# ApsaraDB/galaxysql

Hardware: AMD Instinct MI355X
Metric: probe_rows_per_s (higher is better)
Workload: dtype int64; 1 GPU; C3_tpch_sf100_q3_join_chain_groupby; customer_rows_per_gpu=15000000, orders_rows_per_gpu=150000000, lineitem_rows_scanned_per_gpu=600000000, lineitem_rows_joined_per_gpu=323601457, groups_last_step=12883243, aggregates=SUM(revenue) f64 + SUM(rev_scaled4) i64 + COUNT(*), exchange=none, parallelism=hash_shuffle_dp1, probe_launches=81

## Files before the change

### galaxysql_amd/csrc/gxhip_agg.inc

```

namespace {

struct __align__(16) AggSlot {
    unsigned long long claim;
    uint32_t gid;
    uint32_t pad;
};

__device__ __host__ static inline uint32_t agg_tag(int32_t h) {
    return ((uint32_t)h << 1) | 1u;
}

struct __align__(16) PackedKey {
    unsigned long long lo, hi;
};

__global__ void k_agg_pack(KeyViews keys, int64_t n, int64_t base,
                           PackedKey *packed, uint8_t *nullmask,
                           int32_t *hashes) {
    for (int64_t r = blockIdx.x * (int64_t)blockDim.x + threadIdx.x; r < n;
         r += (int64_t)gridDim.x * blockDim.x) {
        PackedKey p;
        p.lo = 0; p.hi = 0;
        uint8_t mask = 0;
// ... 103 lines not shown
    DevColView input[GX_MAX_COLS];
    unsigned long long *records;
};

struct AggVal {
    unsigned long long bits;
    int32_t type;
    bool isnull;
};

__device__ static inline int64_t aggval_i64(const AggVal &v) {
    return (int64_t)v.bits;
}
__device__ static inline double aggval_f64(const AggVal &v) {
    return v.type == GX_F64 ? __builtin_bit_cast(double, v.bits)
                            : (double)(int64_t)v.bits;
}

__device__ static inline AggVal agg_load(int32_t func, const DevColView &c,
                                         int64_t r) {
    AggVal v;
    v.bits = 0;
    v.type = c.type;
    v.isnull = false;
    if (func == GX_AGG_COUNT_ROW) return v;
    v.isnull = col_is_null(c, r);
    if (v.isnull || func == GX_AGG_COUNT_COL || c.type == GX_SLICE) return v;
    v.bits = c.type == GX_I32
        ? (unsigned long long)(int64_t)((const int32_t *)c.values)[r]
        : ((const unsigned long long *)c.values)[r];
    return v;
}

__device__ static inline void agg_rmw(int32_t func, unsigned long long *rec,
                                      int32_t val_off, int32_t seen_off,
                                      const AggVal &v) {
    unsigned long long *vp = rec + val_off;
    if (func == GX_AGG_COUNT_ROW) {
        atomicAdd(vp, 1ull);
        return;
    }
    if (v.isnull) return;
    switch (func) {
    case GX_AGG_COUNT_COL:
        atomicAdd(vp, 1ull);
        break;
    case GX_AGG_SUM_I64:
        atomicAdd(vp, v.bits);
        break;
    case GX_AGG_SUM_I64N:
        atomicAdd(vp, v.bits);
        if (seen_off >= 0) rec[seen_off] = 1ull;
        break;
    case GX_AGG_SUM_F64:
        atomicAdd((double *)vp, aggval_f64(v));
        rec[seen_off] = 1ull;
        break;
    case GX_AGG_MIN_I64:
        atomic_min_i64((long long *)vp, (long long)aggval_i64(v));
        rec[seen_off] = 1ull;
        break;
    case GX_AGG_MAX_I64:
        atomic_max_i64((long long *)vp, (long long)aggval_i64(v));
        rec[seen_off] = 1ull;
        break;
    case GX_AGG_MIN_F64:
        atomic_jmin_f64(vp, __builtin_bit_cast(double, v.bits));
        rec[seen_off] = 1ull;
        break;
    case GX_AGG_MAX_F64:
        atomic_jmax_f64(vp, __builtin_bit_cast(double, v.bits));
        rec[seen_off] = 1ull;
        break;
    case GX_AGG_BIT_AND: atomicAnd(vp, v.bits); break;
    case GX_AGG_BIT_OR: atomicOr(vp, v.bits); break;
    case GX_AGG_BIT_XOR: atomicXor(vp, v.bits); break;
    case GX_AGG_AVG_F64:
        atomicAdd((double *)vp, aggval_f64(v));
        atomicAdd(rec + seen_off, 1ull);
        break;
    }
}

__device__ static inline void agg_apply(const AggAccumParams &P, uint32_t gid,
                                        int64_t r) {
    unsigned long long *rec = P.records + (size_t)gid * P.stride;
    for (int a = 0; a < P.n_aggs; a++)
        agg_rmw(P.func[a], rec, P.val_off[a], P.seen_off[a],
                agg_load(P.func[a], P.input[a], r));
}

struct AggInsertParams {
    AggSlot *slots;
    uint32_t mask;
    int use_packed;
    const PackedKey *packed;
    const uint8_t *nullmask;
    KeyViews keystore;
    const int32_t *hashes;
    int64_t base_krow;
    int64_t n;
    uint32_t *overflow;
    int inline_gid;
    uint32_t *ngroups;
    uint32_t *krow_of_gid;
    uint32_t *slot_of_gid;
    uint32_t *slot_of_row;
    int fuse_accum;
    int only_failed;
    AggAccumParams A;
};

#define GX_SLOT_FAIL 0xFFFFFFFFu

__device__ static inline bool agg_rows_equal(const AggInsertParams &P,
                                             int64_t a, int64_t b) {
    if (P.use_packed) return packed_equal(P.packed, P.nullmask, a, b);
    return rows_key_equal(P.keystore, a, P.keystore, b);
}

#define GX_GID_PENDING 0xFFFFFFFFu

__global__ void k_agg_insert(AggInsertParams P) {
    for (int64_t r = blockIdx.x * (int64_t)blockDim.x + threadIdx.x; r < P.n;
         r += (int64_t)gridDim.x * blockDim.x) {
        if (P.only_failed && P.slot_of_row[r] != GX_SLOT_FAIL)
            continue;
        const int64_t krow = P.base_krow + r;
        const uint32_t tag = agg_tag(P.hashes[r]);
        const unsigned long long claim =
            ((unsigned long long)tag << 32) | (uint32_t)(krow + 1);
        uint32_t slot = (uint32_t)gx_mix(P.hashes[r]) & P.mask;
        uint32_t probes = 0;
        bool failed = false;
        while (true) {
            unsigned long long old = P.slots[slot].claim;
            if (old == 0ull)
                old = atomicCAS(&P.slots[slot].claim, 0ull, claim);
            if (old == 0ull) {
                if (P.inline_gid) {
                    uint32_t gid = atomicAdd(P.ngroups, 1u);
                    P.slots[slot].gid = gid;
                    P.krow_of_gid[gid] = (uint32_t)krow;
                    if (P.slot_of_gid)
                        P.slot_of_gid[gid] = slot;
                } else {
                    P.slots[slot].gid = GX_GID_PENDING;
                }
                break;
            }
            if ((uint32_t)(old >> 32) == tag) {
                int64_t owner = (int64_t)(uint32_t)old - 1;
                if (agg_rows_equal(P, owner, krow))
                    break;
            }
            if (++probes > (P.mask < 1023u ? P.mask : 1023u)) {
                *P.overflow = 1u;
                failed = true;
                break;
            }
            slot = (slot + 1) & P.mask;
        }
        if (P.fuse_accum) {
            P.slot_of_row[r] = failed ? GX_SLOT_FAIL : slot;
            if (!failed) agg_apply(P.A, slot, r);
        } else {
// ... 990 lines not shown
```

### galaxysql_amd/csrc/gxhip_groupjoin.inc

```

namespace {

struct __align__(16) GJWideEntry {
    int64_t key;
    uint32_t pos;
    uint32_t used;
    unsigned long long s[2];
};

__global__ void k_gjw_expand(const JoinEntry *entries, int64_t n,
                             DevColView keycol, GJWideEntry *wide,
                             unsigned long long s0, unsigned long long s1) {
    for (int64_t i = blockIdx.x * (int64_t)blockDim.x + threadIdx.x; i < n;
         i += (int64_t)gridDim.x * blockDim.x) {
        JoinEntry e = entries[i];
        GJWideEntry w;
        w.key = ((const int64_t *)keycol.values)[e.pos];
        w.pos = e.pos;
        w.used = 0;
        w.s[0] = s0;
        w.s[1] = s1;
        wide[i] = w;
    }
}
// ... 59 lines not shown
__global__ void k_gjw_unpack(const GJWideEntry *wide, int64_t n,
                             unsigned long long *records, int32_t stride,
                             int32_t off0, int32_t off1, int32_t n_aggs,
                             uint32_t *used) {
    for (int64_t i = blockIdx.x * (int64_t)blockDim.x + threadIdx.x; i < n;
         i += (int64_t)gridDim.x * blockDim.x) {
        GJWideEntry w = wide[i];
        unsigned long long *rec = records + (size_t)w.pos * stride;
        rec[off0] = w.s[0];
        if (n_aggs > 1) rec[off1] = w.s[1];
        if (w.used) atomicOr(&used[w.pos >> 5], 1u << (w.pos & 31));
    }
}

struct GJProbeParams {
    const uint32_t *starts;
    const JoinEntry *entries;
    uint32_t mask;
    int64_t n;
    const int32_t *hashes;
    int fast_i64;
    KeyViews build_keys, probe_keys;
    uint32_t *used;
    unsigned long long *matches;
    AggAccumParams A;
};

__global__ void k_gj_probe(GJProbeParams P) {
    uint32_t n_match = 0;
    for (int64_t i = blockIdx.x * (int64_t)blockDim.x + threadIdx.x; i < P.n;
         i += (int64_t)gridDim.x * blockDim.x) {
        uint32_t b = (uint32_t)gx_mix(P.hashes[i]) & P.mask;
        uint32_t it = P.starts[b], end = P.starts[b + 1];
        int64_t want_key = 0;
        if (P.fast_i64)
            want_key = ((const int64_t *)P.probe_keys.col[0].values)[i];
        for (; it < end; it++) {
            JoinEntry e = P.entries[it];
            bool is_match;
            if (P.fast_i64)
                is_match = (e.key == want_key);
            else
                is_match = ((int32_t)e.key == P.hashes[i]) &&
                           rows_key_equal(P.build_keys, e.pos,
                                          P.probe_keys, i);
            if (!is_match) continue;
            n_match++;
            uint32_t w = 1u << (e.pos & 31);
            if ((P.used[e.pos >> 5] & w) == 0)
                atomicOr(&P.used[e.pos >> 5], w);
            agg_apply(P.A, e.pos, i);
        }
    }
    gj_count_matches(P.matches, n_match);
}

struct GJInlineProbeParams {
    const JoinEntry *table;
    const JoinEntry *entries;
    uint32_t mask;
    int64_t n;
    DevColView probe_key;
    uint32_t *used;
    unsigned long long *matches;
    AggAccumParams A;
};

__global__ void k_gj_probe_inline(GJInlineProbeParams P) {
    uint32_t n_match = 0;
    for (int64_t i = blockIdx.x * (int64_t)blockDim.x + threadIdx.x; i < P.n;
         i += (int64_t)gridDim.x * blockDim.x) {
        if (col_is_null(P.probe_key, i)) continue;
        const int64_t want = ((const int64_t *)P.probe_key.values)[i];
        const uint64_t ebase =
            (uint64_t)((uint32_t)gx_mix(gx_hash_i64(want)) & P.mask) * 4;
        const uint32_t end = P.table[ebase].pad;
        const uint32_t ovf0 = end > 4 ? P.table[ebase + 1].pad : 0u;
        for (uint32_t it = 0; it < end; it++) {
            const JoinEntry e = it < 4 ? P.table[ebase + it]
                                       : P.entries[ovf0 + (it - 4)];
            if (e.key != want) continue;
            n_match++;
            uint32_t w = 1u << (e.pos & 31);
            if ((P.used[e.pos >> 5] & w) == 0)
                atomicOr(&P.used[e.pos >> 5], w);
            agg_apply(P.A, e.pos, i);
        }
    }
    gj_count_matches(P.matches, n_match);
}

__global__ void k_gj_compact(const uint32_t *used, int64_t n, uint32_t *out,
                             uint32_t *counter) {
    __shared__ uint32_t s_rows[4][GX_EMIT_STAGE];
    const int wid = threadIdx.x >> 6;
    const int lane = threadIdx.x & 63;
    uint32_t *stage = s_rows[wid];
    uint32_t cnt = 0;

    auto flush = [&]() {
        if (cnt == 0) return;
        uint32_t base = 0;
        if (lane == 0) base = atomicAdd(counter, cnt);
        base = (uint32_t)__shfl((int)base, 0, 64);
        for (uint32_t k = (uint32_t)lane; k < cnt; k += 64)
            out[base + k] = stage[k];
        cnt = 0;
    };

    const int64_t stride = (int64_t)gridDim.x * blockDim.x;
    for (int64_t i = blockIdx.x * (int64_t)blockDim.x + threadIdx.x;;
         i += stride) {
        bool active = i < n;
        if (!__ballot(active)) break;
        bool want = active && (used[i >> 5] >> (i & 31)) & 1u;
        unsigned long long m = __ballot(want);
        uint32_t add = (uint32_t)__popcll(m);
        if (cnt + add > GX_EMIT_STAGE) flush();
        if (want)
            stage[cnt + (uint32_t)__popcll(m & ((1ull << lane) - 1ull))] =
                (uint32_t)i;
        cnt += add;
    }
    flush();
}

__global__ void k_gj_emit(const unsigned long long *records, int32_t stride,
                          int32_t val_off, int32_t seen_off, int32_t func,
                          const uint32_t *idx, const uint32_t *used,
                          int count_row_null_row, int64_t n,
                          void *out_vals, uint8_t *out_nulls) {
    for (int64_t i = blockIdx.x * (int64_t)blockDim.x + threadIdx.x; i < n;
         i += (int64_t)gridDim.x * blockDim.x) {
        uint32_t g = idx ? idx[i] : (uint32_t)i;
        const unsigned long long *rec = records + (size_t)g * stride;
        bool matched = (used[g >> 5] >> (g & 31)) & 1u;
        bool isnull = seen_off >= 0 && rec[seen_off] == 0ull;
        out_nulls[i] = isnull;
        bool f64 = func == GX_AGG_SUM_F64 || func == GX_AGG_MIN_F64 ||
                   func == GX_AGG_MAX_F64 || func == GX_AGG_AVG_F64;
        unsigned long long v = isnull ? 0ull : rec[val_off];
        if (func == GX_AGG_AVG_F64) {
            ((double *)out_vals)[i] = isnull ? 0.0
                : __builtin_bit_cast(double, v) / (double)rec[seen_off];
        } else if (f64) {
            ((double *)out_vals)[i] = isnull ? 0.0
                : __builtin_bit_cast(double, v);
        } else {
            int64_t x = (int64_t)v;
            if (func == GX_AGG_COUNT_ROW && !matched && count_row_null_row)
                x += 1;
            ((int64_t *)out_vals)[i] = x;
        }
    }
}

struct GJEmitParams {
    const unsigned long long *records;
    int32_t stride;
    const uint32_t *idx;
    const uint32_t *used;
    int count_row_null_row;
    int64_t n;
    int32_t n_keys, n_aggs;
    DevColView key_src[GX_MAX_COLS];
    int32_t key_words[GX_MAX_COLS];
    void *key_vals[GX_MAX_COLS];
    uint8_t *key_nulls[GX_MAX_COLS];
    int32_t func[GX_MAX_COLS];
    int32_t val_off[GX_MAX_COLS];
    int32_t seen_off[GX_MAX_COLS];
    void *agg_vals[GX_MAX_COLS];
    uint8_t *agg_nulls[GX_MAX_COLS];
};

__global__ void k_gj_emit_all(GJEmitParams P) {
    for (int64_t i = blockIdx.x * (int64_t)blockDim.x + threadIdx.x; i < P.n;
         i += (int64_t)gridDim.x * blockDim.x) {
        const uint32_t g = P.idx ? P.idx[i] : (uint32_t)i;
        for (int k = 0; k < P.n_keys; k++) {
            const DevColView &src = P.key_src[k];
            const bool nn = col_is_null(src, g);
            if (P.key_nulls[k]) P.key_nulls[k][i] = nn;
            const int32_t w = P.key_words[k];
            const uint32_t *sv = (const uint32_t *)src.values + (size_t)g * w;
            uint32_t *dv = (uint32_t *)P.key_vals[k] + (size_t)i * w;
            for (int32_t j = 0; j < w; j++) dv[j] = nn ? 0u : sv[j];
        }
        const unsigned long long *rec = P.records + (size_t)g * P.stride;
        const bool matched = (P.used[g >> 5] >> (g & 31)) & 1u;
        for (int a = 0; a < P.n_aggs; a++) {
            const int32_t func = P.func[a], so = P.seen_off[a];
            const unsigned long long seen = so >= 0 ? rec[so] : 1ull;
            const bool isnull = seen == 0ull;
            if (P.agg_nulls[a]) P.agg_nulls[a][i] = isnull;
            const unsigned long long v = isnull ? 0ull : rec[P.val_off[a]];
            if (func == GX_AGG_AVG_F64) {
                ((double *)P.agg_vals[a])[i] = isnull ? 0.0
                    : __builtin_bit_cast(double, v) / (double)seen;
            } else if (func == GX_AGG_COUNT_ROW) {
                ((int64_t *)P.agg_vals[a])[i] = (int64_t)v +
                    ((!matched && P.count_row_null_row) ? 1 : 0);
            } else {
                ((unsigned long long *)P.agg_vals[a])[i] = v;
            }
        }
    }
}

struct GroupJoinOp : gx_op {
    gx_groupjoin_cfg cfg;
    std::vector<gx_equi_key> keys;
    std::vector<int32_t> build_types, probe_types, group_cols_;
    std::vector<gx_agg_spec> aggs;

    DevBuf d_accum;
    DevBuf d_wide;
    DevBuf d_pn, d_ph, d_gj_tmp, d_cnt, d_gidx, d_used, d_records;
    DevBuf d_meta;
    std::unique_ptr<JoinOp> jop;
    hipEvent_t ev0 = nullptr, ev1 = nullptr;
    double kernel_ms = 0.0;
    int64_t rows_total = 0, probe_launches = 0, matches_total = 0;
    int32_t stride = 0;
    int32_t val_off[GX_MAX_COLS] = {0};
    int32_t seen_off[GX_MAX_COLS] = {0};
    unsigned long long tmpl[2 * GX_MAX_COLS] = {0};
    bool built = false, emitted = false;
    bool wide_ok = false;
    bool wide = false;
    bool inline_ok = false;
    bool inline_tab = false;

    GroupJoinOp(const gx_groupjoin_cfg *c)
        : gx_op(OP_GROUPJOIN, c->device, c->stream), cfg(*c) {
        keys.assign(c->keys, c->keys + c->n_keys);
        build_types.assign(c->build_types, c->build_types + c->n_build_cols);
        probe_types.assign(c->probe_types, c->probe_types + c->n_probe_cols);
        group_cols_.assign(c->group_cols, c->group_cols + c->n_group_cols);
        aggs.assign(c->aggs, c->aggs + c->n_aggs);

        gx_join_cfg jc{};
        jc.join_type = GX_JOIN_INNER;
        jc.n_keys = (int32_t)keys.size();
        swapped_keys = keys;
        for (auto &k : swapped_keys) std::swap(k.outer_index, k.inner_index);
        jc.keys = swapped_keys.data();
        jc.n_outer_cols = (int32_t)probe_types.size();
        jc.outer_types = probe_types.data();
        jc.n_inner_cols = (int32_t)build_types.size();
        jc.inner_types = build_types.data();
        jc.anti_null_col = -1;
        jc.device = device;
        jc.stream = (uint64_t)stream;
        jc.expected_build_rows = c->expected_build_rows;
        jc.enable_bloom = 1;
        jop.reset(new JoinOp(&jc));
        jop->null_safe_keys = true;

        int32_t off = 0;
        for (size_t a = 0; a < aggs.size(); a++) {
            val_off[a] = off;
            switch (aggs[a].func) {
            case GX_AGG_MIN_I64: tmpl[off] = (unsigned long long)INT64_MAX; break;
            case GX_AGG_MAX_I64: tmpl[off] = (unsigned long long)INT64_MIN; break;
            case GX_AGG_MIN_F64: tmpl[off] = __builtin_bit_cast(unsigned long long, (double)INFINITY); break;
            case GX_AGG_MAX_F64: tmpl[off] = __builtin_bit_cast(unsigned long long, (double)-INFINITY); break;
            case GX_AGG_BIT_AND: tmpl[off] = ~0ull; break;
            default: tmpl[off] = 0ull; break;
            }
            off++;
            bool tracks_null = !(aggs[a].func == GX_AGG_COUNT_ROW ||
                                 aggs[a].func == GX_AGG_COUNT_COL ||
                                 aggs[a].func == GX_AGG_SUM_I64 ||
                                 aggs[a].func == GX_AGG_BIT_AND ||
                                 aggs[a].func == GX_AGG_BIT_OR ||
                                 aggs[a].func == GX_AGG_BIT_XOR);
            if (tracks_null) {
                seen_off[a] = off;
                tmpl[off] = 0ull;
                off++;
            } else {
                seen_off[a] = -1;
            }
        }
        stride = off > 0 ? off : 1;
        wide_ok = keys.size() == 1 && keys[0].unified_type == GX_I64 &&
                  aggs.size() <= 2;
        for (auto &a : aggs)
            wide_ok &= a.func == GX_AGG_COUNT_ROW ||
                       a.func == GX_AGG_COUNT_COL ||
                       a.func == GX_AGG_SUM_I64;
        inline_ok = !wide_ok && keys.size() == 1 &&
                    keys[0].unified_type == GX_I64 &&
                    build_types[keys[0].outer_index] == GX_I64 &&
                    probe_types[keys[0].inner_index] == GX_I64;
    }
    std::vector<gx_equi_key> swapped_keys;

    ~GroupJoinOp() override {
        if (ev0) (void)hipEventDestroy(ev0);
        if (ev1) (void)hipEventDestroy(ev1);
    }

    int consume(const gx_chunk *ch) { return jop->consume(ch); }

    int do_build() {
        inline_tab = inline_ok && jop->build.n_rows > 0 &&
                     !jop->build.cols[jop->build_key_cols[0]].has_nulls;
        jop->null_safe_keys = !inline_tab;
        if (jop->do_build()) return -1;
        const int64_t n = jop->build.n_rows;
        if (d_meta.grow(16, stream)) return -1;
        HIP_OK(hipMemsetAsync(d_meta.p, 0, 16, stream));
        if (n > 0) {
            if (d_records.grow((size_t)n * stride * 8, stream)) return -1;
            AggInitParams P;
            P.records = (unsigned long long *)d_records.p;
            P.stride = stride;
            P.from = 0;
            P.to = n;
            std::memcpy(P.tmpl, tmpl, sizeof(tmpl));
            hipLaunchKernelGGL(k_agg_init, dim3(gx_grid(n * stride)),
                               dim3(256), 0, stream, P);
        }
        size_t words = (size_t)((n + 31) / 32);
        if (words == 0) words = 1;
        if (d_used.grow(words * 4, stream)) return -1;
        HIP_OK(hipMemsetAsync(d_used.p, 0, words * 4, stream));
        wide = wide_ok && n > 0 &&
               !jop->build.cols[jop->build_key_cols[0]].has_nulls;
        if (wide) {
            if (d_wide.grow((size_t)n * sizeof(GJWideEntry), stream))
                return -1;
            hipLaunchKernelGGL(k_gjw_expand, dim3(gx_grid(n)), dim3(256), 0,
                               stream, (const JoinEntry *)jop->d_entries.p, n,
                               jop->build.view(jop->build_key_cols[0]),
                               (GJWideEntry *)d_wide.p, tmpl[val_off[0]],
                               aggs.size() > 1 ? tmpl[val_off[1]] : 0ull);
        }
        built = true;
        return 0;
    }

    int probe(const gx_chunk *ch) {
        if (!built) { gx_set_err("probe before build"); return -1; }
        if (ensure_device(device)) return -1;
        if (jop->pass_nothing || ch->n_rows == 0) return 0;
        StagedChunk st;
        if (st.stage(ch, stream)) return -1;
        const int64_t n = st.n_rows;
        KeyViews pk = jop->key_views_staged(st, jop->probe_key_cols);
        if (!inline_tab) {
            if (d_ph.grow((size_t)n * 4, stream) ||
                d_pn.grow((size_t)n, stream)) return -1;
            hipLaunchKernelGGL(k_hash_rows, dim3(gx_grid(n)), dim3(256), 0,
                               stream, pk, n, (int32_t *)d_ph.p,
                               (uint8_t *)d_pn.p, 1 );
        }
        if (!ev0) {
            HIP_OK(hipEventCreate(&ev0));
            HIP_OK(hipEventCreate(&ev1));
        }
        if (inline_tab) {
            GJInlineProbeParams P;
            std::memset(&P, 0, sizeof(P));
            P.table = (const JoinEntry *)jop->d_table.p;
            P.entries = (const JoinEntry *)jop->d_entries.p;
            P.mask = jop->mask;
            P.n = n;
            P.probe_key = pk.col[0];
            P.used = (uint32_t *)d_used.p;
            P.matches = (unsigned long long *)d_meta.p;
            fill_accum(P.A, st);
            HIP_OK(hipEventRecord(ev0, stream));
            hipLaunchKernelGGL(k_gj_probe_inline, dim3(gx_grid(n)), dim3(256),
                               0, stream, P);
        } else if (wide) {
            GJWideProbeParams W;
            std::memset(&W, 0, sizeof(W));
            W.matches = (unsigned long long *)d_meta.p;
            W.starts = (const uint32_t *)jop->d_starts.p;
            W.wide = (GJWideEntry *)d_wide.p;
            W.mask = jop->mask;
            W.n = n;
            W.hashes = (const int32_t *)d_ph.p;
            W.probe_key = pk.col[0];
            W.n_aggs = (int32_t)aggs.size();
            for (size_t a = 0; a < aggs.size(); a++) {
                W.func[a] = aggs[a].func;
                if (aggs[a].input_col >= 0)
                    W.input[a] = st.views[aggs[a].input_col];
            }
            HIP_OK(hipEventRecord(ev0, stream));
            hipLaunchKernelGGL(k_gjw_probe, dim3(gx_grid(n)), dim3(256),
                               0, stream, W);
        } else {
            GJProbeParams P;
            std::memset(&P, 0, sizeof(P));
            P.starts = (const uint32_t *)jop->d_starts.p;
            P.entries = (const JoinEntry *)jop->d_entries.p;
            P.mask = jop->mask;
            P.n = n;
            P.hashes = (const int32_t *)d_ph.p;
            P.fast_i64 = (int)jop->fast_i64;
            P.build_keys = jop->key_views(jop->build, jop->build_key_cols);
            P.probe_keys = pk;
            P.used = (uint32_t *)d_used.p;
            P.matches = (unsigned long long *)d_meta.p;
            fill_accum(P.A, st);
            HIP_OK(hipEventRecord(ev0, stream));
            hipLaunchKernelGGL(k_gj_probe, dim3(gx_grid(n)), dim3(256), 0,
                               stream, P);
        }
        HIP_OK(hipEventRecord(ev1, stream));
        if (finish_probe(nullptr)) return -1;
        rows_total += n;
        return 0;
    }

    void fill_accum(AggAccumParams &A, const StagedChunk &st) const {
        A.n_aggs = (int32_t)aggs.size();
        A.stride = stride;
        for (size_t a = 0; a < aggs.size(); a++) {
            A.func[a] = aggs[a].func;
            A.val_off[a] = val_off[a];
            A.seen_off[a] = seen_off[a];
            if (aggs[a].input_col >= 0)
                A.input[a] = st.views[aggs[a].input_col];
        }
        A.records = (unsigned long long *)d_records.p;
    }

    int finish_probe(int64_t *kept) {
        struct { unsigned long long matches; uint32_t kept, pad; } meta;
        HIP_OK(hipMemcpyAsync(&meta, d_meta.p, 16, hipMemcpyDeviceToHost,
                              stream));
        HIP_OK(hipStreamSynchronize(stream));
        float ms = 0;
        HIP_OK(hipEventElapsedTime(&ms, ev0, ev1));
        kernel_ms += ms;
        probe_launches++;
        matches_total = (int64_t)meta.matches;
        if (kept) *kept = meta.kept;
        return 0;
    }

    int next(gx_result **out) {
        *out = nullptr;
        if (!built) { gx_set_err("next before build"); return -1; }
        if (emitted || jop->pass_nothing) return 0;
        if (ensure_device(device)) return -1;
        emitted = true;
        const int64_t n_build = jop->build.n_rows;
        if (n_build == 0) return 0;
        if (wide) {
            hipLaunchKernelGGL(k_gjw_unpack, dim3(gx_grid(n_build)), dim3(256),
                               0, stream, (const GJWideEntry *)d_wide.p,
                               n_build, (unsigned long long *)d_records.p,
                               stride, val_off[0],
                               aggs.size() > 1 ? val_off[1] : 0,
                               (int32_t)aggs.size(), (uint32_t *)d_used.p);
        }

        const bool emit_all = cfg.join_type == GX_JOIN_LEFT;
        int64_t n_emit = n_build;
        const uint32_t *idx = nullptr;
        if (!emit_all) {
            if (d_gidx.grow((size_t)n_build * 4, stream) ||
                d_cnt.grow(4, stream)) return -1;
            HIP_OK(hipMemsetAsync(d_cnt.p, 0, 4, stream));
            hipLaunchKernelGGL(k_gj_compact, dim3(gx_grid(n_build)), dim3(256),
                               0, stream, (const uint32_t *)d_used.p, n_build,
                               (uint32_t *)d_gidx.p, (uint32_t *)d_cnt.p);
            uint32_t cnt = 0;
            HIP_OK(hipMemcpyAsync(&cnt, d_cnt.p, 4, hipMemcpyDeviceToHost,
                                  stream));
            HIP_OK(hipStreamSynchronize(stream));
            n_emit = cnt;
            idx = (const uint32_t *)d_gidx.p;
        }
        if (n_emit == 0) return 0;

        std::vector<int32_t> otypes;
        for (int32_t gc : group_cols_) otypes.push_back(build_types[gc]);
        for (auto &sp : aggs) {
            switch (sp.func) {
            case GX_AGG_COUNT_ROW: case GX_AGG_COUNT_COL:
            case GX_AGG_SUM_I64: case GX_AGG_SUM_I64N:
            case GX_AGG_MIN_I64: case GX_AGG_MAX_I64:
            case GX_AGG_BIT_AND: case GX_AGG_BIT_OR: case GX_AGG_BIT_XOR:
                otypes.push_back(GX_I64); break;
            default: otypes.push_back(GX_F64); break;
            }
        }
        bool fixed_width = group_cols_.size() <= GX_MAX_COLS;
        for (int32_t gc : group_cols_)
            if (build_types[gc] == GX_SLICE) fixed_width = false;
        if (fixed_width) {
            std::vector<uint8_t> null_free;
            for (int32_t gc : group_cols_)
                null_free.push_back(!jop->build.view(gc).has_nulls);
            for (size_t a = 0; a < aggs.size(); a++)
                null_free.push_back(seen_off[a] < 0);
            auto h = alloc_result_cols(otypes, n_emit, device, stream,
                                       &null_free);
            if (!h) return -1;
            GJEmitParams E;
            std::memset(&E, 0, sizeof(E));
            E.records = (const unsigned long long *)d_records.p;
            E.stride = stride;
            E.idx = idx;
            E.used = (const uint32_t *)d_used.p;
            E.count_row_null_row = (int)emit_all;
            E.n = n_emit;
            E.n_keys = (int32_t)group_cols_.size();
            E.n_aggs = (int32_t)aggs.size();
            size_t col = 0;
            for (size_t k = 0; k < group_cols_.size(); k++, col++) {
                E.key_src[k] = jop->build.view(group_cols_[k]);
                E.key_words[k] =
                    (int32_t)(gx_fixed_size(build_types[group_cols_[k]]) / 4);
                E.key_vals[k] = h->bufs[col * 2].p;
                E.key_nulls[k] = (uint8_t *)h->bufs[col * 2 + 1].p;
            }
            for (size_t a = 0; a < aggs.size(); a++, col++) {
                E.func[a] = aggs[a].func;
                E.val_off[a] = val_off[a];
                E.seen_off[a] = seen_off[a];
                E.agg_vals[a] = h->bufs[col * 2].p;
                E.agg_nulls[a] = (uint8_t *)h->bufs[col * 2 + 1].p;
            }
            hipLaunchKernelGGL(k_gj_emit_all, dim3(gx_grid(n_emit)),
                               dim3(256), 0, stream, E);
            HIP_OK(hipStreamSynchronize(stream));
            give_result(std::move(h), out);
            return 0;
        }
        auto h = alloc_result_cols(otypes, n_emit, device, stream);
        if (!h) return -1;
        if (emit_all) {
            if (d_gidx.grow((size_t)n_build * 4, stream)) return -1;
            hipLaunchKernelGGL(k_iota, dim3(gx_grid(n_build)), dim3(256), 0,
                               stream, (uint32_t *)d_gidx.p, n_build);
            idx = (const uint32_t *)d_gidx.p;
        }
        size_t col = 0;
        for (int32_t gc : group_cols_) {
            DevColView src = jop->build.view(gc);
            if (src.type == GX_SLICE) {
                if (gather_slice_col(src, idx, 0, n_emit, h.get(), col,
                                     d_gj_tmp, stream))
                    return -1;
            } else {
                hipLaunchKernelGGL(k_gather, dim3(gx_grid(n_emit)), dim3(256),
                                   0, stream, src, idx, n_emit,
                                   h->bufs[col * 2].p,
                                   (uint8_t *)h->bufs[col * 2 + 1].p, 0);
            }
            col++;
        }
        for (size_t a = 0; a < aggs.size(); a++) {
            hipLaunchKernelGGL(k_gj_emit, dim3(gx_grid(n_emit)), dim3(256), 0,
                               stream, (const unsigned long long *)d_records.p,
                               stride, val_off[a], seen_off[a], aggs[a].func,
                               emit_all ? nullptr : idx,
                               (const uint32_t *)d_used.p, (int)emit_all,
                               n_emit, h->bufs[col * 2].p,
                               (uint8_t *)h->bufs[col * 2 + 1].p);
            col++;
        }
        HIP_OK(hipStreamSynchronize(stream));
        give_result(std::move(h), out);
        return 0;
    }
};

}

extern "C" {

gx_op *gxop_groupjoin_create(const gx_groupjoin_cfg *cfg) {
    if (cfg)
        for (int32_t i = 0; i < cfg->n_aggs; i++)
            if (gx_agg_is_distinct(cfg->aggs[i].func)) {
                gx_set_err("DISTINCT aggregates are gxop_agg only "
                           "(not supported in group-join)");
                return nullptr;
            }
    if (cfg)
        for (int32_t i = 0; i < cfg->n_aggs; i++)
            if (cfg->aggs[i].func == GX_AGG_RANK ||
                cfg->aggs[i].func == GX_AGG_DENSE_RANK) {
                gx_set_err("RANK/DENSE_RANK are window-only");
                return nullptr;
            }
    if (!cfg || cfg->n_keys <= 0 || cfg->n_keys > GX_MAX_KEYS ||
        (cfg->join_type != GX_JOIN_INNER && cfg->join_type != GX_JOIN_LEFT) ||
        cfg->n_aggs > GX_MAX_COLS) {
        gx_set_err("bad groupjoin cfg");
        return nullptr;
    }
    if (cfg->device < 0) { gx_set_err("gxhip requires a GPU device"); return nullptr; }
    HIP_OK_NULL(hipSetDevice(cfg->device));
    return new GroupJoinOp(cfg);
}
int gxop_groupjoin_consume(gx_op *op, const gx_chunk *c) {
    if (!op || op->kind != OP_GROUPJOIN) { gx_set_err("not a groupjoin op"); return -1; }
    return static_cast<GroupJoinOp *>(op)->consume(c);
}
int gxop_groupjoin_build(gx_op *op) {
    if (!op || op->kind != OP_GROUPJOIN) { gx_set_err("not a groupjoin op"); return -1; }
    return static_cast<GroupJoinOp *>(op)->do_build();
}
int gxop_groupjoin_probe(gx_op *op, const gx_chunk *c) {
    if (!op || op->kind != OP_GROUPJOIN) { gx_set_err("not a groupjoin op"); return -1; }
    return static_cast<GroupJoinOp *>(op)->probe(c);
}
int gxop_groupjoin_next(gx_op *op, gx_result **out) {
    if (!op || op->kind != OP_GROUPJOIN) { gx_set_err("not a groupjoin op"); return -1; }
    return static_cast<GroupJoinOp *>(op)->next(out);
}
int gxop_groupjoin_close(gx_op *op) { delete op; return 0; }
int gxop_groupjoin_get_stats(gx_op *op, gx_join_stats *out) {
    if (!op || op->kind != OP_GROUPJOIN || !out) { gx_set_err("not a groupjoin op"); return -1; }
    GroupJoinOp *g = static_cast<GroupJoinOp *>(op);
    out->probe_kernel_ms = g->kernel_ms;
    out->probe_launches = g->probe_launches;
    out->probe_rows = g->rows_total;
    out->matches = g->matches_total;
    return 0;
}

}
```

### galaxysql_amd/csrc/gxhip_scan.inc

```

namespace {

#define GX_MAX_PREDS 8

struct ScanPreds {
    int32_t n_preds;
    int32_t pred_cmp[GX_MAX_PREDS];
    int64_t pred_i64[GX_MAX_PREDS];
    double  pred_f64[GX_MAX_PREDS];
    const uint8_t *pred_pat[GX_MAX_PREDS];
    int32_t pred_plen[GX_MAX_PREDS];
    DevColView pred_view[GX_MAX_PREDS];
};

struct ScanParams {
    int64_t n;
    ScanPreds preds;
    int32_t n_projs;
    int32_t proj_op[GX_MAX_COLS];
    int32_t proj_scale[GX_MAX_COLS];
    DevColView proj_a[GX_MAX_COLS];
    DevColView proj_b[GX_MAX_COLS];
    DevColView proj_c[GX_MAX_COLS];
    DevColView proj_d[GX_MAX_COLS];
// ... 315 lines not shown
        int64_t key[GX_PS_R];
        uint32_t pass = 0, knull = 0;
#pragma unroll
        for (int r = 0; r < GX_PS_R; r++) {
            const int64_t row = row0 + r * 64;
            const bool in = row < n;
            key[r] = in ? keys[row] : 0;
            if (in) pass |= 1u << r;
            if (kc.has_nulls && in && kc.nulls[row]) knull |= 1u << r;
        }
        if (wide) {
            pass = scan_rows_pass_wide(S, row0, n, pass);
        } else {
#pragma unroll
            for (int r = 0; r < GX_PS_R; r++)
                if (((pass >> r) & 1u) && !scan_row_passes(S, row0 + r * 64))
                    pass &= ~(1u << r);
        }
#pragma unroll
        for (int r = 0; r < GX_PS_R; r++)
            n_kept += (uint32_t)__popcll(__ballot((pass >> r) & 1u));

        uint32_t live = pass & ~knull;
        if (bloom) {
            uint64_t word[GX_PS_R], bits[GX_PS_R];
#pragma unroll
            for (int r = 0; r < GX_PS_R; r++) {
                const uint64_t x = bloom_mix(key[r]);
                bits[r] = bloom_bits(x);
                word[r] = ((live >> r) & 1u)
                    ? bloom[bloom_word(x, P.bloom_mask)] : 0ull;
            }
#pragma unroll
            for (int r = 0; r < GX_PS_R; r++)
                if ((word[r] & bits[r]) != bits[r]) live &= ~(1u << r);
        }

#pragma unroll
        for (int r = 0; r < GX_PS_R; r++) {
            const bool want = (live >> r) & 1u;
            const unsigned long long m = __ballot(want);
            if (want) {
                const uint32_t at = qcnt + (uint32_t)__popcll(m & lt_mask);
                qkey[at] = key[r];
                qrow[at] = (uint32_t)(row0 + r * 64);
            }
            qcnt += (uint32_t)__popcll(m);
        }

        while (qcnt >= 64) {
            qcnt -= 64;
            probe_key<GX_PS_STAGE>(P, E, true, qrow[qcnt + lane],
                                   qkey[qcnt + lane], flush);
        }
    }
    if (qcnt) {
        const bool active = (uint32_t)lane < qcnt;
        probe_key<GX_PS_STAGE>(P, E, active, active ? qrow[lane] : 0u,
                               active ? qkey[lane] : 0, flush);
    }
    flush(P, E);
    if (lane == 0 && n_kept) atomicAdd(kept, n_kept);
}

__global__ void __launch_bounds__(256)
k_probe_scan(ProbeParams P, ScanPreds S, uint32_t *kept) {
    probe_scan_body(P, S, kept, PairListFlush());
}

struct GJAccum {
    int32_t n_aggs;
    int32_t stride;
    int32_t func[GX_MAX_COLS];
    int32_t val_off[GX_MAX_COLS];
    int32_t seen_off[GX_MAX_COLS];
    int32_t op[GX_MAX_COLS];
    DevColView a[GX_MAX_COLS];
    DevColView b[GX_MAX_COLS];
    DevColView c[GX_MAX_COLS];
    DevColView d[GX_MAX_COLS];
    unsigned long long *records;
    uint32_t *used;
    unsigned long long *matches;
};

struct AccumFlush {
    const GJAccum *A;
    __device__ inline void operator()(const ProbeParams &,
                                      EmitStage &E) const {
        if (E.cnt == 0) return;
        const GJAccum &G = *A;
        for (uint32_t i = (uint32_t)E.lane; i < E.cnt; i += 64) {
            const int64_t row = E.s_p[i];
            const uint32_t pos = E.s_b[i];
            const uint32_t w = 1u << (pos & 31);
            if ((G.used[pos >> 5] & w) == 0)
                atomicOr(&G.used[pos >> 5], w);
            unsigned long long *rec = G.records + (size_t)pos * G.stride;
            for (int a = 0; a < G.n_aggs; a++) {
                AggVal v;
                v.bits = 0;
                v.type = GX_I64;
                v.isnull = false;
                if (G.func[a] != GX_AGG_COUNT_ROW)
                    v = proj_value(G.op[a], G.a[a], G.b[a], G.c[a], G.d[a],
                                   row);
                agg_rmw(G.func[a], rec, G.val_off[a], G.seen_off[a], v);
            }
        }
        if (E.lane == 0) atomicAdd(G.matches, (unsigned long long)E.cnt);
        E.cnt = 0;
    }
};

__global__ void __launch_bounds__(256)
k_gj_probe_scan(ProbeParams P, ScanPreds S, uint32_t *kept,
                const GJAccum *A) {
    AccumFlush flush;
    flush.A = A;
    probe_scan_body(P, S, kept, flush);
}

struct ProjGatherParams {
    const uint32_t *pidx;
    const uint32_t *bidx;
    int64_t n;
    int32_t n_cols;
    int32_t side[GX_MAX_COLS];
    int32_t op[GX_MAX_COLS];
    int32_t scale[GX_MAX_COLS];
    DevColView a[GX_MAX_COLS];
    DevColView b[GX_MAX_COLS];
    DevColView c[GX_MAX_COLS];
    DevColView d[GX_MAX_COLS];
    void *out_vals[GX_MAX_COLS];
    uint8_t *out_nulls[GX_MAX_COLS];
};

__global__ void k_gather_proj(ProjGatherParams G) {
    for (int64_t i = blockIdx.x * (int64_t)blockDim.x + threadIdx.x; i < G.n;
         i += (int64_t)gridDim.x * blockDim.x) {
        const int64_t pi = G.pidx[i];
        const int64_t bi = G.bidx[i];
        for (int c = 0; c < G.n_cols; c++)
            proj_store(G.op[c], G.scale[c], G.a[c], G.b[c], G.c[c], G.d[c],
                       G.side[c] ? bi : pi, G.out_vals[c], G.out_nulls[c], i,
                       nullptr);
    }
}

__global__ void k_scan(ScanParams P) {
    __shared__ uint32_t s_rows[4][GX_EMIT_STAGE];
    const int wid = threadIdx.x >> 6;
    const int lane = threadIdx.x & 63;
    uint32_t *stage = s_rows[wid];
    uint32_t cnt = 0;

    auto flush = [&]() {
        if (cnt == 0) return;
        uint32_t base = 0;
        if (lane == 0) base = atomicAdd(P.counter, cnt);
        base = (uint32_t)__shfl((int)base, 0, 64);
        for (uint32_t k = (uint32_t)lane; k < cnt; k += 64) {
            uint32_t at = base + k;
            if (at >= P.cap) continue;
            int64_t src = stage[k];
            if (P.out_rowids) P.out_rowids[at] = (uint32_t)src;
            for (int c = 0; c < P.n_projs; c++)
                proj_store(P.proj_op[c], P.proj_scale[c], P.proj_a[c],
                           P.proj_b[c], P.proj_c[c], P.proj_d[c], src,
                           P.out_vals[c], P.out_nulls[c], at, P.err);
        }
        cnt = 0;
    };

    const int64_t stride = (int64_t)gridDim.x * blockDim.x;
    for (int64_t base_i = blockIdx.x * (int64_t)blockDim.x + threadIdx.x;;
         base_i += stride) {
        bool active = base_i < P.n;
// ... 282 lines not shown
            HIP_OK(hipStreamSynchronize(stream));
        }
        give_result(std::move(h), out);
        return 0;
    }
    return -1;
}


bool gj_probe_scan_fast_ok(const GroupJoinOp *g, const ScanOp *s,
                           const gx_chunk *raw) {
    if (!g->inline_tab || g->jop->pass_nothing) return false;
    if (raw->n_rows <= 0 || (int64_t)raw->n_rows >= (INT64_C(1) << 31) ||
        raw->n_blocks != (int32_t)s->input_types.size())
        return false;
    for (int32_t b = 0; b < raw->n_blocks; b++)
        if (raw->blocks[b].mem != GX_MEM_DEVICE) return false;
    const gx_proj &kp = s->projs[(size_t)g->jop->probe_key_cols[0]];
    if (kp.op != GX_PROJ_COPY || s->input_types[kp.a] != GX_I64) return false;
    for (auto &pr : s->projs)
        if (pr.op == GX_PROJ_DEC_TO_SCALED) return false;
    for (auto &sp : g->aggs) {
        if (sp.input_col < 0) continue;
        const gx_proj &pr = s->projs[(size_t)sp.input_col];
        const int32_t t = s->out_types[(size_t)sp.input_col];
        switch (pr.op) {
        case GX_PROJ_COPY:
            if (t != GX_I64 && t != GX_I32 && t != GX_F64) return false;
            break;
        case GX_PROJ_REV_F64: case GX_PROJ_REV_SCALED4:
        case GX_PROJ_Q9_AMOUNT4:
            break;
        default:
            return false;
        }
    }
    return true;
}

int gj_probe_scan_fused(GroupJoinOp *g, ScanOp *s, const gx_chunk *raw,
                        int64_t *n_kept) {
    if (ensure_device(g->device)) return -1;
    hipStream_t stream = g->stream;
    JoinOp *j = g->jop.get();
    StagedChunk st;
    if (st.stage(raw, stream)) return -1;
    const int64_t n = st.n_rows;
    ScanPreds S;
    if (s->fill_preds(S, st)) return -1;
    const gx_proj &kp = s->projs[(size_t)j->probe_key_cols[0]];

    ProbeParams P;
    std::memset(&P, 0, sizeof(P));
    P.table = (const JoinEntry *)j->d_table.p;
    P.entries = (const JoinEntry *)j->d_entries.p;
    P.mask = j->mask;
    P.n_probe = n;
    P.bloom = (const uint32_t *)j->d_bloom.p;
    P.bloom_mask = j->bloom_mask;
    P.fast_i64 = 1;
    P.probe_keys.n = 1;
    P.probe_keys.col[0] = st.views[kp.a];
    P.join_type = GX_JOIN_INNER;
    P.anti_null_col = -1;

    GJAccum A;
    std::memset(&A, 0, sizeof(A));
    A.n_aggs = (int32_t)g->aggs.size();
    A.stride = g->stride;
    for (size_t a = 0; a < g->aggs.size(); a++) {
        A.func[a] = g->aggs[a].func;
        A.val_off[a] = g->val_off[a];
        A.seen_off[a] = g->seen_off[a];
        if (g->aggs[a].input_col < 0) continue;
        const gx_proj &pr = s->projs[(size_t)g->aggs[a].input_col];
        A.op[a] = pr.op;
        A.a[a] = st.views[pr.a];
        if (pr.op != GX_PROJ_COPY) A.b[a] = st.views[pr.b];
        if (pr.op == GX_PROJ_Q9_AMOUNT4) {
            A.c[a] = st.views[pr.c];
            A.d[a] = st.views[pr.d];
        }
    }
    A.records = (unsigned long long *)g->d_records.p;
    A.used = (uint32_t *)g->d_used.p;
    A.matches = (unsigned long long *)g->d_meta.p;
    if (g->d_accum.grow(sizeof(A), stream)) return -1;
    HIP_OK(hipMemcpyAsync(g->d_accum.p, &A, sizeof(A), hipMemcpyHostToDevice,
                          stream));
    HIP_OK(hipMemsetAsync((char *)g->d_meta.p + 8, 0, 4, stream));
    if (!g->ev0) {
        HIP_OK(hipEventCreate(&g->ev0));
        HIP_OK(hipEventCreate(&g->ev1));
    }
    HIP_OK(hipEventRecord(g->ev0, stream));
    hipLaunchKernelGGL(k_gj_probe_scan, dim3(gx_ps_grid(n)), dim3(256), 0,
                       stream, P, S, (uint32_t *)g->d_meta.p + 2,
                       (const GJAccum *)g->d_accum.p);
    HIP_OK(hipEventRecord(g->ev1, stream));
    if (g->finish_probe(n_kept)) return -1;
    g->rows_total += *n_kept;
    return 0;
}

}

extern "C" {

int gxop_groupjoin_probe_scan(gx_op *groupjoin, gx_op *scan,
                              const gx_chunk *raw_chunk,
                              int64_t *n_scan_kept, int64_t *n_matched) {
    if (!groupjoin || groupjoin->kind != OP_GROUPJOIN) { gx_set_err("not a groupjoin op"); return -1; }
    if (!scan || scan->kind != OP_SCAN) { gx_set_err("not a scan op"); return -1; }
    if (!raw_chunk) { gx_set_err("groupjoin_probe_scan: null argument"); return -1; }
    if (groupjoin->device != scan->device || groupjoin->stream != scan->stream) {
        gx_set_err("groupjoin_probe_scan: group-join and scan must share "
                   "device and stream");
        return -1;
    }
    GroupJoinOp *g = static_cast<GroupJoinOp *>(groupjoin);
    ScanOp *s = static_cast<ScanOp *>(scan);
    std::lock_guard<std::mutex> lk(groupjoin->mu);
    if (g->probe_types != s->out_types) {
        gx_set_err("groupjoin_probe_scan: scan's projected types differ "
                   "from the group-join's probe_types");
        return -1;
    }
    if (!g->built) { gx_set_err("probe before build"); return -1; }
    const int64_t before = g->matches_total;
    int64_t kept = 0;
    int rc;
    if (gj_probe_scan_fast_ok(g, s, raw_chunk)) {
        rc = gj_probe_scan_fused(g, s, raw_chunk, &kept);
    } else {
        gx_result *t = nullptr;
        rc = s->consume(raw_chunk, &t);
        if (rc) return rc;
        kept = t->chunk.n_rows;
        rc = g->probe(&t->chunk);
        gxop_result_release(t);
    }
    if (rc) return rc;
    if (n_scan_kept) *n_scan_kept = kept;
    if (n_matched) *n_matched = g->matches_total - before;
    return 0;
}

int gxop_join_probe_scan(gx_op *join, gx_op *scan, const gx_chunk *raw_chunk,
                         gx_result **out, int64_t *n_scan_kept) {
    if (!join || join->kind != OP_JOIN) { gx_set_err("not a join op"); return -1; }
    if (!scan || scan->kind != OP_SCAN) { gx_set_err("not a scan op"); return -1; }
    if (!raw_chunk || !out) { gx_set_err("probe_scan: null argument"); return -1; }
    *out = nullptr;
    if (join->device != scan->device || join->stream != scan->stream) {
        gx_set_err("probe_scan: join and scan must share device and stream");
        return -1;
    }
    ScanOp *s = static_cast<ScanOp *>(scan);
    std::lock_guard<std::mutex> lk(join->mu);
    JoinOp *j = join->variant == 0 ? static_cast<JoinOp *>(join) : nullptr;
    HybridJoinOp *hj = j ? nullptr : static_cast<HybridJoinOp *>(join);
    const gx_join_cfg &cfg = j ? j->cfg : hj->cfg;
    const std::vector<int32_t> &pt = cfg.build_outer
        ? (j ? j->inner_types : hj->inner_types)
        : (j ? j->outer_types : hj->outer_types);
    if (pt != s->out_types) {
        gx_set_err("probe_scan: scan's projected types differ from the "
                   "join's probe-side types");
// ... 56 lines not shown
```

Before: 18.61 billion rows/s.

## Transpose group-join aggregate atomics across lanes and replace used bitmap with COUNT slot

For additive aggregates whose record fits in four 64-bit slots, the probe flush now gathers each row's deltas into registers. It then transposes them across lanes with shuffles, so neighbouring lanes issue atomics to neighbouring slots of the same record instead of each lane updating a whole record on its own. This is meant to turn scattered per-lane atomic sequences into coalesced atomic instructions on shared cache lines. For inner joins with a COUNT(*) aggregate, the matched-row bitmap is dropped and compaction and emit test the count slot instead, which removes one extra read/atomicOr per match. The cost is more shuffles and ballots per flush batch and a more complex code path.

```diff
diff --git a/galaxysql_amd/csrc/gxhip_agg.inc b/galaxysql_amd/csrc/gxhip_agg.inc
--- a/galaxysql_amd/csrc/gxhip_agg.inc
+++ b/galaxysql_amd/csrc/gxhip_agg.inc
@@ -209,6 +209,90 @@
     }
 }
 
+#define GX_AGG_T_SLOTS 4
+
+__host__ __device__ static inline bool agg_func_additive(int32_t func) {
+    return func == GX_AGG_COUNT_ROW || func == GX_AGG_COUNT_COL ||
+           func == GX_AGG_SUM_I64 || func == GX_AGG_SUM_I64N ||
+           func == GX_AGG_SUM_F64 || func == GX_AGG_AVG_F64;
+}
+__host__ __device__ static inline bool agg_func_adds_f64(int32_t func) {
+    return func == GX_AGG_SUM_F64 || func == GX_AGG_AVG_F64;
+}
+
+struct AggSlotOps {
+    unsigned long long v[GX_AGG_T_SLOTS];
+    uint32_t skip;
+};
+
+__device__ static inline void agg_slot_ops_clear(AggSlotOps &o) {
+#pragma unroll
+    for (int s = 0; s < GX_AGG_T_SLOTS; s++) o.v[s] = 0ull;
+    o.skip = (1u << GX_AGG_T_SLOTS) - 1u;
+}
+
+__device__ static inline void agg_slot_ops_put(AggSlotOps &o, int32_t func,
+                                               int32_t val_off,
+                                               int32_t seen_off,
+                                               const AggVal &v) {
+    if (func != GX_AGG_COUNT_ROW && v.isnull) return;
+    unsigned long long x = v.bits;
+    if (func == GX_AGG_COUNT_ROW || func == GX_AGG_COUNT_COL) x = 1ull;
+    else if (agg_func_adds_f64(func))
+        x = __builtin_bit_cast(unsigned long long, aggval_f64(v));
+#pragma unroll
+    for (int s = 0; s < GX_AGG_T_SLOTS; s++) {
+        if (s == val_off) { o.v[s] = x; o.skip &= ~(1u << s); }
+        if (s == seen_off) { o.v[s] = 1ull; o.skip &= ~(1u << s); }
+    }
+}
+
+__device__ static inline void agg_add_transposed(unsigned long long *records,
+                                                 int32_t stride, int32_t width,
+                                                 uint32_t f64_slots,
+                                                 uint32_t rec_index,
+                                                 AggSlotOps o, int lane) {
+    unsigned long long skip_of[GX_AGG_T_SLOTS];
+#pragma unroll
+    for (int s = 0; s < GX_AGG_T_SLOTS; s++)
+        skip_of[s] = __ballot((o.skip >> s) & 1u);
+#pragma unroll
+    for (int b = 1; b < GX_AGG_T_SLOTS; b <<= 1) {
+        const bool hi = (lane & b) != 0;
+#pragma unroll
+        for (int r = 0; r < GX_AGG_T_SLOTS; r++) {
+            if ((r & b) == 0 && (r | b) < width) {
+                const unsigned long long got =
+                    __shfl_xor(hi ? o.v[r] : o.v[r | b], b, 64);
+                if (hi) o.v[r] = got;
+                else o.v[r | b] = got;
+            }
+        }
+    }
+    const int slot = lane & (width - 1);
+    const int lane0 = lane - slot;
+    unsigned long long my_skip = skip_of[0];
+#pragma unroll
+    for (int s = 1; s < GX_AGG_T_SLOTS; s++)
+        if (slot == s) my_skip = skip_of[s];
+    const bool f64 = (f64_slots >> slot) & 1u;
+    uint32_t at[GX_AGG_T_SLOTS];
+#pragma unroll
+    for (int i = 0; i < GX_AGG_T_SLOTS; i++)
+        at[i] = (uint32_t)__shfl((int)rec_index,
+                                 lane0 + (i < width ? i : 0), 64);
+#pragma unroll
+    for (int i = 0; i < GX_AGG_T_SLOTS; i++) {
+        if (i < width && !((my_skip >> (lane0 + i)) & 1ull)) {
+            unsigned long long *w = records + (size_t)at[i] * stride + slot;
+            if (f64)
+                atomicAdd((double *)w, __builtin_bit_cast(double, o.v[i]));
+            else
+                atomicAdd(w, o.v[i]);
+        }
+    }
+}
+
 __device__ static inline void agg_apply(const AggAccumParams &P, uint32_t gid,
                                         int64_t r) {
     unsigned long long *rec = P.records + (size_t)gid * P.stride;
diff --git a/galaxysql_amd/csrc/gxhip_groupjoin.inc b/galaxysql_amd/csrc/gxhip_groupjoin.inc
--- a/galaxysql_amd/csrc/gxhip_groupjoin.inc
+++ b/galaxysql_amd/csrc/gxhip_groupjoin.inc
@@ -165,7 +165,7 @@
             if (e.key != want) continue;
             n_match++;
             uint32_t w = 1u << (e.pos & 31);
-            if ((P.used[e.pos >> 5] & w) == 0)
+            if (P.used && (P.used[e.pos >> 5] & w) == 0)
                 atomicOr(&P.used[e.pos >> 5], w);
             agg_apply(P.A, e.pos, i);
         }
@@ -173,8 +173,10 @@
     gj_count_matches(P.matches, n_match);
 }
 
-__global__ void k_gj_compact(const uint32_t *used, int64_t n, uint32_t *out,
-                             uint32_t *counter) {
+__global__ void k_gj_compact(const uint32_t *used,
+                             const unsigned long long *records,
+                             int32_t rec_stride, int32_t count_off,
+                             int64_t n, uint32_t *out, uint32_t *counter) {
     __shared__ uint32_t s_rows[4][GX_EMIT_STAGE];
     const int wid = threadIdx.x >> 6;
     const int lane = threadIdx.x & 63;
@@ -196,7 +198,11 @@
          i += stride) {
         bool active = i < n;
         if (!__ballot(active)) break;
-        bool want = active && (used[i >> 5] >> (i & 31)) & 1u;
+        bool want = false;
+        if (active)
+            want = count_off >= 0
+                ? records[(size_t)i * rec_stride + count_off] != 0ull
+                : (used[i >> 5] >> (i & 31)) & 1u;
         unsigned long long m = __ballot(want);
         uint32_t add = (uint32_t)__popcll(m);
         if (cnt + add > GX_EMIT_STAGE) flush();
@@ -211,13 +217,15 @@
 __global__ void k_gj_emit(const unsigned long long *records, int32_t stride,
                           int32_t val_off, int32_t seen_off, int32_t func,
                           const uint32_t *idx, const uint32_t *used,
-                          int count_row_null_row, int64_t n,
+                          int32_t count_off, int count_row_null_row,
+                          int64_t n,
                           void *out_vals, uint8_t *out_nulls) {
     for (int64_t i = blockIdx.x * (int64_t)blockDim.x + threadIdx.x; i < n;
          i += (int64_t)gridDim.x * blockDim.x) {
         uint32_t g = idx ? idx[i] : (uint32_t)i;
         const unsigned long long *rec = records + (size_t)g * stride;
-        bool matched = (used[g >> 5] >> (g & 31)) & 1u;
+        bool matched = count_off >= 0 ? rec[count_off] != 0ull
+                                      : (used[g >> 5] >> (g & 31)) & 1u;
         bool isnull = seen_off >= 0 && rec[seen_off] == 0ull;
         out_nulls[i] = isnull;
         bool f64 = func == GX_AGG_SUM_F64 || func == GX_AGG_MIN_F64 ||
@@ -243,6 +251,7 @@
     int32_t stride;
     const uint32_t *idx;
     const uint32_t *used;
+    int32_t count_off;
     int count_row_null_row;
     int64_t n;
     int32_t n_keys, n_aggs;
@@ -271,7 +280,9 @@
             for (int32_t j = 0; j < w; j++) dv[j] = nn ? 0u : sv[j];
         }
         const unsigned long long *rec = P.records + (size_t)g * P.stride;
-        const bool matched = (P.used[g >> 5] >> (g & 31)) & 1u;
+        const bool matched = P.count_off >= 0
+            ? rec[P.count_off] != 0ull
+            : (P.used[g >> 5] >> (g & 31)) & 1u;
         for (int a = 0; a < P.n_aggs; a++) {
             const int32_t func = P.func[a], so = P.seen_off[a];
             const unsigned long long seen = so >= 0 ? rec[so] : 1ull;
@@ -314,6 +325,7 @@
     bool wide = false;
     bool inline_ok = false;
     bool inline_tab = false;
+    int32_t count_off = -1;
 
     GroupJoinOp(const gx_groupjoin_cfg *c)
         : gx_op(OP_GROUPJOIN, c->device, c->stream), cfg(*c) {
@@ -392,6 +404,10 @@
         inline_tab = inline_ok && jop->build.n_rows > 0 &&
                      !jop->build.cols[jop->build_key_cols[0]].has_nulls;
         jop->null_safe_keys = !inline_tab;
+        count_off = -1;
+        if (inline_tab && cfg.join_type == GX_JOIN_INNER)
+            for (size_t a = 0; a < aggs.size() && count_off < 0; a++)
+                if (aggs[a].func == GX_AGG_COUNT_ROW) count_off = val_off[a];
         if (jop->do_build()) return -1;
         const int64_t n = jop->build.n_rows;
         if (d_meta.grow(16, stream)) return -1;
@@ -453,7 +469,7 @@
             P.mask = jop->mask;
             P.n = n;
             P.probe_key = pk.col[0];
-            P.used = (uint32_t *)d_used.p;
+            P.used = count_off >= 0 ? nullptr : (uint32_t *)d_used.p;
             P.matches = (unsigned long long *)d_meta.p;
             fill_accum(P.A, st);
             HIP_OK(hipEventRecord(ev0, stream));
@@ -554,7 +570,9 @@
                 d_cnt.grow(4, stream)) return -1;
             HIP_OK(hipMemsetAsync(d_cnt.p, 0, 4, stream));
             hipLaunchKernelGGL(k_gj_compact, dim3(gx_grid(n_build)), dim3(256),
-                               0, stream, (const uint32_t *)d_used.p, n_build,
+                               0, stream, (const uint32_t *)d_used.p,
+                               (const unsigned long long *)d_records.p,
+                               stride, count_off, n_build,
                                (uint32_t *)d_gidx.p, (uint32_t *)d_cnt.p);
             uint32_t cnt = 0;
             HIP_OK(hipMemcpyAsync(&cnt, d_cnt.p, 4, hipMemcpyDeviceToHost,
@@ -595,6 +613,7 @@
             E.stride = stride;
             E.idx = idx;
             E.used = (const uint32_t *)d_used.p;
+            E.count_off = count_off;
             E.count_row_null_row = (int)emit_all;
             E.n = n_emit;
             E.n_keys = (int32_t)group_cols_.size();
@@ -648,7 +667,8 @@
                                stream, (const unsigned long long *)d_records.p,
                                stride, val_off[a], seen_off[a], aggs[a].func,
                                emit_all ? nullptr : idx,
-                               (const uint32_t *)d_used.p, (int)emit_all,
+                               (const uint32_t *)d_used.p, count_off,
+                               (int)emit_all,
                                n_emit, h->bufs[col * 2].p,
                                (uint8_t *)h->bufs[col * 2 + 1].p);
             col++;
diff --git a/galaxysql_amd/csrc/gxhip_scan.inc b/galaxysql_amd/csrc/gxhip_scan.inc
--- a/galaxysql_amd/csrc/gxhip_scan.inc
+++ b/galaxysql_amd/csrc/gxhip_scan.inc
@@ -421,6 +421,8 @@
     unsigned long long *records;
     uint32_t *used;
     unsigned long long *matches;
+    int32_t t_width;
+    uint32_t t_f64;
 };
 
 struct AccumFlush {
@@ -429,11 +431,43 @@
                                       EmitStage &E) const {
         if (E.cnt == 0) return;
         const GJAccum &G = *A;
+        if (G.t_width) {
+            for (uint32_t i0 = 0; i0 < E.cnt; i0 += 64) {
+                const uint32_t i = i0 + (uint32_t)E.lane;
+                const bool active = i < E.cnt;
+                const int64_t row = active ? (int64_t)E.s_p[i] : 0;
+                const uint32_t pos = active ? E.s_b[i] : 0u;
+                const uint32_t w = 1u << (pos & 31);
+                uint32_t seen_w = w;
+                if (G.used && active) seen_w = G.used[pos >> 5];
+                AggSlotOps o;
+                agg_slot_ops_clear(o);
+#pragma unroll
+                for (int a = 0; a < GX_AGG_T_SLOTS; a++) {
+                    if (a >= G.n_aggs || !active) continue;
+                    AggVal v;
+                    v.bits = 0;
+                    v.type = GX_I64;
+                    v.isnull = false;
+                    if (G.func[a] != GX_AGG_COUNT_ROW)
+                        v = proj_value(G.op[a], G.a[a], G.b[a], G.c[a],
+                                       G.d[a], row);
+                    agg_slot_ops_put(o, G.func[a], G.val_off[a],
+                                     G.seen_off[a], v);
+                }
+                if ((seen_w & w) == 0) atomicOr(&G.used[pos >> 5], w);
+                agg_add_transposed(G.records, G.stride, G.t_width, G.t_f64,
+                                   pos, o, E.lane);
+            }
+            if (E.lane == 0) atomicAdd(G.matches, (unsigned long long)E.cnt);
+            E.cnt = 0;
+            return;
+        }
         for (uint32_t i = (uint32_t)E.lane; i < E.cnt; i += 64) {
             const int64_t row = E.s_p[i];
             const uint32_t pos = E.s_b[i];
             const uint32_t w = 1u << (pos & 31);
-            if ((G.used[pos >> 5] & w) == 0)
+            if (G.used && (G.used[pos >> 5] & w) == 0)
                 atomicOr(&G.used[pos >> 5], w);
             unsigned long long *rec = G.records + (size_t)pos * G.stride;
             for (int a = 0; a < G.n_aggs; a++) {
@@ -882,8 +916,17 @@
             A.d[a] = st.views[pr.d];
         }
     }
+    bool additive = g->stride <= GX_AGG_T_SLOTS;
+    for (size_t a = 0; a < g->aggs.size(); a++)
+        additive = additive && agg_func_additive(g->aggs[a].func);
+    if (additive) {
+        A.t_width = g->stride <= 1 ? 1 : g->stride == 2 ? 2 : 4;
+        for (size_t a = 0; a < g->aggs.size(); a++)
+            if (agg_func_adds_f64(g->aggs[a].func))
+                A.t_f64 |= 1u << g->val_off[a];
+    }
     A.records = (unsigned long long *)g->d_records.p;
-    A.used = (uint32_t *)g->d_used.p;
+    A.used = g->count_off >= 0 ? nullptr : (uint32_t *)g->d_used.p;
     A.matches = (unsigned long long *)g->d_meta.p;
     if (g->d_accum.grow(sizeof(A), stream)) return -1;
     HIP_OK(hipMemcpyAsync(g->d_accum.p, &A, sizeof(A), hipMemcpyHostToDevice,
```

After: 21.15 billion rows/s (median of 6 runs). 1.14x the previous value.
